# ANRGUSC/DEFER

Hardware: NVIDIA H100
Metric: inferences_per_sec (higher is better)
Workload: dtype bf16x3->f32

## Files before the change

### defer_b200/csrc/conv_umma.cu

```cuda
#include <cuda.h>
#include <string.h>

#include <type_traits>

#include <vector>

#include "common.cuh"
#include "conv_umma.cuh"

namespace defer {

static int env_int(const char* name, int dflt) {
  const char* v = getenv(name);
  return v ? atoi(v) : dflt;
}

namespace {

constexpr int BM = 128;
constexpr int BK = 64;
constexpr int CONS_THREADS = 256;
constexpr int NUM_THREADS = CONS_THREADS + 128;
constexpr int SMEM_CAP = 227 * 1024 - 256;
constexpr int CTL_BYTES = 256;
constexpr int MAX_STAGES = 8;
constexpr int MEGA_BN = 64;
constexpr int STG_COLS = 64;
constexpr int STG_BYTES = BM * STG_COLS * 4;

struct KParams {
  int n, ho, wo, cout;
  int tile_n, tile_h, tile_w, tiles_h, tiles_w;
  int flat;
  int m_total;
  int kh, kw, sh, sw, pad_t, pad_l;
  int cblocks;
  int k_blocks;
  int splits;
  int cluster;
  uint32_t flags;
  const float* scale;
  const float* shift;
  const void* res;
  void* y;
  float* partial;
  unsigned int* counters;
  size_t plane_out;
};

struct alignas(128) MegaOp {
  CUtensorMap tmx[2];
  CUtensorMap tmw[2];
  KParams p;
  int m_tiles, n_tiles;
  const float* stem_x;
  int stem_h, stem_w, stem_cin, stem_kh, stem_kw, stem_sh, stem_sw, stem_pad_t, stem_pad_l, stem_K;
  int stem_win_rows, stem_win_cols;
  const uint8_t* stem_u8;
  float stem_shift[3];
  const float* scale2;
  const float* shift2;
  void* y2;
  int relu2;
  int store_first;
};

template <int NPLANES, int BN>
struct Smem {
  static constexpr int A_PLANE = BM * 128;
  static constexpr int B_PLANE = BN * 128;
  static constexpr int STAGE = NPLANES * (A_PLANE + B_PLANE);
  static constexpr int RED = BM * BN * 4;
  __host__ __device__ static constexpr int ring(int stages, bool red) {
    return (red && stages * STAGE < RED) ? RED : stages * STAGE;
  }
  __host__ __device__ static constexpr int total(int stages, bool red) {
    return ring(stages, red) + STG_BYTES + CTL_BYTES + 1024;
  }
  __host__ __device__ static constexpr int max_stages() {
    return (SMEM_CAP - STG_BYTES - CTL_BYTES - 1024) / STAGE > MAX_STAGES ? MAX_STAGES
                                                                          : (SMEM_CAP - STG_BYTES - CTL_BYTES - 1024) / STAGE;
  }
};
static_assert(Smem<2, 128>::max_stages() == 3 && Smem<2, 64>::max_stages() == 4, "BF16X2 ring depths");
static_assert(Smem<1, 64>::max_stages() == 8 && Smem<1, 128>::max_stages() == 6, "BF16 ring depths");

__device__ __forceinline__ uint32_t smem_u32(const void* p) { return (uint32_t)__cvta_generic_to_shared(p); }

__device__ __forceinline__ void mbar_init(uint32_t bar, uint32_t count) {
  asm volatile("mbarrier.init.shared::cta.b64 [%0], %1;" ::"r"(bar), "r"(count));
}
__device__ __forceinline__ void mbar_arrive_expect_tx(uint32_t bar, uint32_t bytes) {
  asm volatile("mbarrier.arrive.expect_tx.shared::cta.b64 _, [%0], %1;" ::"r"(bar), "r"(bytes) : "memory");
}
__device__ __forceinline__ void mbar_expect_tx(uint32_t bar, uint32_t bytes) {
  asm volatile("mbarrier.expect_tx.relaxed.cta.shared::cta.b64 [%0], %1;" ::"r"(bar), "r"(bytes) : "memory");
}
__device__ __forceinline__ void mbar_arrive(uint32_t bar) {
  asm volatile("mbarrier.arrive.shared::cta.b64 _, [%0];" ::"r"(bar) : "memory");
}
__device__ __forceinline__ bool mbar_try_wait(uint32_t bar, uint32_t parity) {
  uint32_t ok;
  asm volatile(
      "{\n.reg .pred p;\n"
      "mbarrier.try_wait.parity.shared::cta.b64 p, [%1], %2;\n"
      "selp.u32 %0, 1, 0, p;\n}\n"
      : "=r"(ok)
      : "r"(bar), "r"(parity)
      : "memory");
  return ok != 0;
}
__device__ __forceinline__ unsigned long long gtimer() {
  unsigned long long t;
  asm volatile("mov.u64 %0, %%globaltimer;" : "=l"(t));
  return t;
}
__device__ int g_conv_wait_timeout_tag;
__device__ __forceinline__ void mbar_wait(uint32_t bar, uint32_t parity, int tag) {
  if (mbar_try_wait(bar, parity)) return;
  unsigned long long t0 = gtimer();
  unsigned spins = 0;
  while (!mbar_try_wait(bar, parity)) {
    if ((++spins & 0xfff) == 0 && gtimer() - t0 > 2000000000ull) {
      g_conv_wait_timeout_tag = tag;
      asm volatile("trap;");
    }
  }
}

__device__ __forceinline__ void tma_load_4d(uint32_t dst, const CUtensorMap* map, uint32_t bar, int c0, int c1, int c2,
                                            int c3) {
  asm volatile(
      "cp.async.bulk.tensor.4d.shared::cluster.global.mbarrier::complete_tx::bytes [%0], [%1, {%3, %4, %5, %6}], [%2];"
      ::"r"(dst), "l"(reinterpret_cast<uint64_t>(map)), "r"(bar), "r"(c0), "r"(c1), "r"(c2), "r"(c3)
      : "memory");
}
__device__ __forceinline__ void tma_load_3d(uint32_t dst, const CUtensorMap* map, uint32_t bar, int c0, int c1, int c2) {
  asm volatile(
      "cp.async.bulk.tensor.3d.shared::cluster.global.mbarrier::complete_tx::bytes [%0], [%1, {%3, %4, %5}], [%2];"
      ::"r"(dst), "l"(reinterpret_cast<uint64_t>(map)), "r"(bar), "r"(c0), "r"(c1), "r"(c2)
      : "memory");
}

__device__ __forceinline__ void cluster_sync_all() {
  asm volatile("barrier.cluster.arrive.release.aligned;" ::: "memory");
  asm volatile("barrier.cluster.wait.acquire.aligned;" ::: "memory");
}
__device__ __forceinline__ uint32_t cluster_ctarank() {
  uint32_t r;
  asm volatile("mov.u32 %0, %%cluster_ctarank;" : "=r"(r));
  return r;
}
__device__ __forceinline__ uint32_t cluster_nctarank() {
  uint32_t r;
  asm volatile("mov.u32 %0, %%cluster_nctarank;" : "=r"(r));
  return r;
}
__device__ __forceinline__ uint32_t dsmem_map(uint32_t local_addr, uint32_t rank) {
  uint32_t r;
  asm volatile("mapa.shared::cluster.u32 %0, %1, %2;" : "=r"(r) : "r"(local_addr), "r"(rank));
  return r;
}
__device__ __forceinline__ float4 dsmem_ld4(uint32_t addr) {
  float4 v;
  asm volatile("ld.shared::cluster.v4.f32 {%0, %1, %2, %3}, [%4];" : "=f"(v.x), "=f"(v.y), "=f"(v.z), "=f"(v.w) : "r"(addr));
  return v;
}
__device__ __forceinline__ void cons_bar_sync() { asm volatile("bar.sync 1, 256;" ::: "memory"); }
__device__ __forceinline__ void prod_bar_sync() { asm volatile("bar.sync 2, 128;" ::: "memory"); }

__device__ __forceinline__ uint64_t make_sw128_desc(uint32_t smem_addr) {
  return (uint64_t)((smem_addr & 0x3FFFF) >> 4) | (1ull << 16) | (64ull << 32) | (1ull << 62);
}
__device__ __forceinline__ void wg_fence() { asm volatile("wgmma.fence.sync.aligned;" ::: "memory"); }
__device__ __forceinline__ void wg_commit() { asm volatile("wgmma.commit_group.sync.aligned;" ::: "memory"); }
template <int N>
__device__ __forceinline__ void wg_wait() {
  asm volatile("wgmma.wait_group.sync.aligned %0;" ::"n"(N) : "memory");
}
template <int R>
__device__ __forceinline__ void acc_fence(float (&d)[R]) {
#pragma unroll
  for (int i = 0; i < R; ++i) asm volatile("" : "+f"(d[i])::"memory");
}

template <int BN>
__device__ __forceinline__ void wgmma_bf16(float (&d)[BN / 2], uint64_t a, uint64_t b);

template <>
__device__ __forceinline__ void wgmma_bf16<64>(float (&d)[32], uint64_t a, uint64_t b) {
  asm volatile(
      "{\n.reg .pred p;\nsetp.ne.b32 p, %34, 0;\n"
      "wgmma.mma_async.sync.aligned.m64n64k16.f32.bf16.bf16 "
      "{%0, %1, %2, %3, %4, %5, %6, %7, %8, %9, %10, %11, %12, %13, %14, %15, %16, %17, %18, %19, %20, %21, %22, "
      "%23, %24, %25, %26, %27, %28, %29, %30, %31}, %32, %33, p, 1, 1, 0, 0;\n}\n"
      : "+f"(d[0]), "+f"(d[1]), "+f"(d[2]), "+f"(d[3]), "+f"(d[4]), "+f"(d[5]), "+f"(d[6]), "+f"(d[7]), "+f"(d[8]),
        "+f"(d[9]), "+f"(d[10]), "+f"(d[11]), "+f"(d[12]), "+f"(d[13]), "+f"(d[14]), "+f"(d[15]), "+f"(d[16]),
        "+f"(d[17]), "+f"(d[18]), "+f"(d[19]), "+f"(d[20]), "+f"(d[21]), "+f"(d[22]), "+f"(d[23]), "+f"(d[24]),
        "+f"(d[25]), "+f"(d[26]), "+f"(d[27]), "+f"(d[28]), "+f"(d[29]), "+f"(d[30]), "+f"(d[31])
      : "l"(a), "l"(b), "r"(1));
}

template <>
__device__ __forceinline__ void wgmma_bf16<128>(float (&d)[64], uint64_t a, uint64_t b) {
  asm volatile(
      "{\n.reg .pred p;\nsetp.ne.b32 p, %66, 0;\n"
      "wgmma.mma_async.sync.aligned.m64n128k16.f32.bf16.bf16 "
      "{%0, %1, %2, %3, %4, %5, %6, %7, %8, %9, %10, %11, %12, %13, %14, %15, %16, %17, %18, %19, %20, %21, %22, "
      "%23, %24, %25, %26, %27, %28, %29, %30, %31, %32, %33, %34, %35, %36, %37, %38, %39, %40, %41, %42, %43, %44, "
      "%45, %46, %47, %48, %49, %50, %51, %52, %53, %54, %55, %56, %57, %58, %59, %60, %61, %62, %63}, %64, %65, p, "
      "1, 1, 0, 0;\n}\n"
      : "+f"(d[0]), "+f"(d[1]), "+f"(d[2]), "+f"(d[3]), "+f"(d[4]), "+f"(d[5]), "+f"(d[6]), "+f"(d[7]), "+f"(d[8]),
        "+f"(d[9]), "+f"(d[10]), "+f"(d[11]), "+f"(d[12]), "+f"(d[13]), "+f"(d[14]), "+f"(d[15]), "+f"(d[16]),
        "+f"(d[17]), "+f"(d[18]), "+f"(d[19]), "+f"(d[20]), "+f"(d[21]), "+f"(d[22]), "+f"(d[23]), "+f"(d[24]),
        "+f"(d[25]), "+f"(d[26]), "+f"(d[27]), "+f"(d[28]), "+f"(d[29]), "+f"(d[30]), "+f"(d[31]), "+f"(d[32]),
        "+f"(d[33]), "+f"(d[34]), "+f"(d[35]), "+f"(d[36]), "+f"(d[37]), "+f"(d[38]), "+f"(d[39]), "+f"(d[40]),
        "+f"(d[41]), "+f"(d[42]), "+f"(d[43]), "+f"(d[44]), "+f"(d[45]), "+f"(d[46]), "+f"(d[47]), "+f"(d[48]),
        "+f"(d[49]), "+f"(d[50]), "+f"(d[51]), "+f"(d[52]), "+f"(d[53]), "+f"(d[54]), "+f"(d[55]), "+f"(d[56]),
        "+f"(d[57]), "+f"(d[58]), "+f"(d[59]), "+f"(d[60]), "+f"(d[61]), "+f"(d[62]), "+f"(d[63])
      : "l"(a), "l"(b), "r"(1));
}

__device__ __forceinline__ void row_to_pixel(const KParams& p, int r, int n0, int h0, int w0, bool& valid, size_t& pix) {
  if (p.flat) {
    const int m = w0 + r;
    valid = m < p.m_total;
    pix = (size_t)m;
  } else {
    const int tw = r % p.tile_w;
    const int t2 = r / p.tile_w;
    const int th = t2 % p.tile_h;
    const int tn = t2 / p.tile_h;
    const int nn = n0 + tn, oh = h0 + th, ow = w0 + tw;
    valid = (tn < p.tile_n) && nn < p.n && oh < p.ho && ow < p.wo;
    pix = ((size_t)nn * p.ho + oh) * p.wo + ow;
  }
}

struct EpiArgs {
  const float* scale;
  const float* shift;
  const __nv_bfloat16* res;
  __nv_bfloat16* y;
  size_t plane;
  int cout;
  bool relu;
  bool store_first;
  bool relu2;
  const float* scale2;
  const float* shift2;
  __nv_bfloat16* y2;
};

__device__ __forceinline__ EpiArgs epi_args(const MegaOp& op) {
  const KParams& p = op.p;
  EpiArgs e;
  e.scale = p.scale;
  e.shift = p.shift;
  e.res = reinterpret_cast<const __nv_bfloat16*>(p.res);
  e.y = reinterpret_cast<__nv_bfloat16*>(p.y);
  e.plane = p.plane_out;
  e.cout = p.cout;
  e.relu = (p.flags & DEFER_FLAG_RELU) != 0;
  e.store_first = op.store_first != 0;
  e.relu2 = op.relu2 != 0;
  e.scale2 = op.scale2;
  e.shift2 = op.shift2;
  e.y2 = reinterpret_cast<__nv_bfloat16*>(op.y2);
  return e;
}

__device__ __forceinline__ uint32_t stg_off(int r, int c) {
  return (uint32_t)(r * STG_COLS + (((c >> 2) ^ ((r & 7) << 1)) << 2) + (c & 3)) * 4u;
}
__device__ __forceinline__ void sts2(uint32_t addr, float a, float b) {
  asm volatile("st.shared.v2.f32 [%0], {%1, %2};" ::"r"(addr), "f"(a), "f"(b));
}
__device__ __forceinline__ float4 lds4(uint32_t addr) {
  float4 v;
  asm volatile("ld.shared.v4.f32 {%0, %1, %2, %3}, [%4];" : "=f"(v.x), "=f"(v.y), "=f"(v.z), "=f"(v.w) : "r"(addr));
  return v;
}
__device__ __forceinline__ void stg4(void* p, uint4 v) {
  asm volatile("st.global.v4.b32 [%0], {%1, %2, %3, %4};" ::"l"(p), "r"(v.x), "r"(v.y), "r"(v.z), "r"(v.w));
}

__device__ __forceinline__ float bf_lo(uint32_t w) { return __uint_as_float(w << 16); }
__device__ __forceinline__ float bf_hi(uint32_t w) { return __uint_as_float(w & 0xffff0000u); }

template <int NPLANES, int BN, bool AFF>
__device__ __forceinline__ void epi_tile(const KParams& p, const EpiArgs& e, uint32_t stg, const float (&acc)[BN / 2],
                                         uint32_t qmask, int c_base, int n0, int h0, int w0) {
  const int tid = threadIdx.x;
  const int lane = tid & 31;
  const int row0 = (tid >> 7) * 64 + ((tid >> 5) & 3) * 16 + (lane >> 2);
  const int col_l = 2 * (lane & 3);
  const int jg = tid & 7;
  const int rb = tid >> 3;
  const int ca = 2 * jg + ((jg >> 2) & 1), cb = ca ^ 1;
  const bool swap = (jg >> 2) & 1;
  size_t orow[4];
  uint32_t vmask = 0;
#pragma unroll
  for (int k = 0; k < 4; ++k) {
    bool v;
    size_t pix;
    row_to_pixel(p, rb + 32 * k, n0, h0, w0, v, pix);
    orow[k] = pix * (size_t)e.cout;
    vmask |= (uint32_t)v << k;
  }
#pragma unroll
  for (int P = 0; P < BN / STG_COLS; ++P) {
    const bool mine = (qmask >> (8 * P + jg)) & 1u;
    const int c = c_base + STG_COLS * P + 8 * jg;
    cons_bar_sync();
#pragma unroll
    for (int qq = 0; qq < 8; ++qq) {
      const int q = 8 * P + qq;
      if (!((qmask >> q) & 1u)) continue;
      sts2(stg + stg_off(row0, 8 * qq + col_l), acc[4 * q], acc[4 * q + 1]);
      sts2(stg + stg_off(row0 + 8, 8 * qq + col_l), acc[4 * q + 2], acc[4 * q + 3]);
    }
    uint4 rh[4], rl[4];
#pragma unroll
    for (int k = 0; k < 4; ++k) {
      rh[k] = rl[k] = make_uint4(0u, 0u, 0u, 0u);
      if (e.res && mine && ((vmask >> k) & 1u)) {
        rh[k] = __ldcg(reinterpret_cast<const uint4*>(e.res + orow[k] + c));
        if (NPLANES == 2) rl[k] = __ldcg(reinterpret_cast<const uint4*>(e.res + e.plane + orow[k] + c));
      }
    }
    float sc[8], sf[8];
#pragma unroll
    for (int i = 0; i < 8; ++i) { sc[i] = 1.f; sf[i] = 0.f; }
    if (mine) {
      if (e.scale) {
        const float4 a = __ldg(reinterpret_cast<const float4*>(e.scale + c));
        const float4 b = __ldg(reinterpret_cast<const float4*>(e.scale + c + 4));
        sc[0] = a.x; sc[1] = a.y; sc[2] = a.z; sc[3] = a.w; sc[4] = b.x; sc[5] = b.y; sc[6] = b.z; sc[7] = b.w;
      }
      if (e.shift) {
        const float4 a = __ldg(reinterpret_cast<const float4*>(e.shift + c));
        const float4 b = __ldg(reinterpret_cast<const float4*>(e.shift + c + 4));
        sf[0] = a.x; sf[1] = a.y; sf[2] = a.z; sf[3] = a.w; sf[4] = b.x; sf[5] = b.y; sf[6] = b.z; sf[7] = b.w;
      }
    }
    cons_bar_sync();
    if (!mine) continue;

#pragma unroll
    for (int k = 0; k < 4; ++k) {
      if (!((vmask >> k) & 1u)) continue;
      const int r = rb + 32 * k;
      const float4 xa = lds4(stg + stg_off(r, 4 * ca));
      const float4 xb = lds4(stg + stg_off(r, 4 * cb));
      const float4 x0 = swap ? xb : xa, x1 = swap ? xa : xb;
      float v[8] = {x0.x, x0.y, x0.z, x0.w, x1.x, x1.y, x1.z, x1.w};
      const uint32_t hw[4] = {rh[k].x, rh[k].y, rh[k].z, rh[k].w};
      const uint32_t lw[4] = {rl[k].x, rl[k].y, rl[k].z, rl[k].w};
#pragma unroll
      for (int i = 0; i < 8; ++i) {
        v[i] = fmaf(v[i], sc[i], sf[i]);
        if (e.res) {
          v[i] += (i & 1) ? bf_hi(hw[i >> 1]) : bf_lo(hw[i >> 1]);
          if (NPLANES == 2) v[i] += (i & 1) ? bf_hi(lw[i >> 1]) : bf_lo(lw[i >> 1]);
        }
        if (e.relu) v[i] = fmaxf(v[i], 0.f);
      }
      uint4 hi, lo = make_uint4(0u, 0u, 0u, 0u);
      if (NPLANES == 2) {
        split_bf16x2(v[0], v[1], hi.x, lo.x);
        split_bf16x2(v[2], v[3], hi.y, lo.y);
        split_bf16x2(v[4], v[5], hi.z, lo.z);
        split_bf16x2(v[6], v[7], hi.w, lo.w);
      } else {
        hi = make_uint4(pack_bf16x2(v[0], v[1]), pack_bf16x2(v[2], v[3]), pack_bf16x2(v[4], v[5]), pack_bf16x2(v[6], v[7]));
      }
      const size_t o = orow[k] + c;
      if (!AFF || e.store_first) {
        stg4(e.y + o, hi);
        if (NPLANES == 2) stg4(e.y + e.plane + o, lo);
      }
      if constexpr (AFF) {
        float s2[8], t2[8];
        {
          const float4 a = __ldg(reinterpret_cast<const float4*>(e.scale2 + c));
          const float4 b = __ldg(reinterpret_cast<const float4*>(e.scale2 + c + 4));
          const float4 d = __ldg(reinterpret_cast<const float4*>(e.shift2 + c));
          const float4 f = __ldg(reinterpret_cast<const float4*>(e.shift2 + c + 4));
          s2[0] = a.x; s2[1] = a.y; s2[2] = a.z; s2[3] = a.w; s2[4] = b.x; s2[5] = b.y; s2[6] = b.z; s2[7] = b.w;
          t2[0] = d.x; t2[1] = d.y; t2[2] = d.z; t2[3] = d.w; t2[4] = f.x; t2[5] = f.y; t2[6] = f.z; t2[7] = f.w;
        }
        const uint32_t sh[4] = {hi.x, hi.y, hi.z, hi.w};
        const uint32_t sl[4] = {lo.x, lo.y, lo.z, lo.w};
        float u[8];
#pragma unroll
        for (int i = 0; i < 8; ++i) {
          u[i] = (i & 1) ? bf_hi(sh[i >> 1]) : bf_lo(sh[i >> 1]);
          if (NPLANES == 2) u[i] = u[i] + ((i & 1) ? bf_hi(sl[i >> 1]) : bf_lo(sl[i >> 1]));
          u[i] = fmaf(u[i], s2[i], t2[i]);
          if (e.relu2) u[i] = fmaxf(u[i], 0.f);
        }
        uint4 h2, l2;
        if (NPLANES == 2) {
          split_bf16x2(u[0], u[1], h2.x, l2.x);
          split_bf16x2(u[2], u[3], h2.y, l2.y);
          split_bf16x2(u[4], u[5], h2.z, l2.z);
          split_bf16x2(u[6], u[7], h2.w, l2.w);
          stg4(e.y2 + o, h2);
          stg4(e.y2 + e.plane + o, l2);
        } else {
          h2 = make_uint4(pack_bf16x2(u[0], u[1]), pack_bf16x2(u[2], u[3]), pack_bf16x2(u[4], u[5]), pack_bf16x2(u[6], u[7]));
          stg4(e.y2 + o, h2);
        }
      }
    }
  }
}

template <int NPLANES, int BN, int MODE, bool AFF = false>
__device__ __forceinline__ void conv_body(const MegaOp* ops, int n_ops, int stages, int pdl) {
  using L = Smem<NPLANES, BN>;
  constexpr int R = BN / 2;
  extern __shared__ uint8_t smem_raw[];
  uint8_t* smem = reinterpret_cast<uint8_t*>((reinterpret_cast<uintptr_t>(smem_raw) + 1023) & ~(uintptr_t)1023);
  const uint32_t ring = smem_u32(smem);
  const bool red = MODE == 0 && ops[0].p.cluster;
  const uint32_t stg = ring + L::ring(stages, red);
  const uint32_t bar_base = stg + STG_BYTES;
  auto full_bar = [&](int s) { return bar_base + 8u * s; };
  auto empty_bar = [&](int s) { return bar_base + 8u * (stages + s); };
  __shared__ int s_is_last;

  const int tid = threadIdx.x;
  if (tid == 0) {
    for (int s = 0; s < stages; ++s) {
      mbar_init(full_bar(s), 1);
      mbar_init(empty_bar(s), CONS_THREADS / 32);
    }
    asm volatile("fence.mbarrier_init.release.cluster;" ::: "memory");
  }
  __syncthreads();
  if (pdl) {
    asm volatile("griddepcontrol.wait;" ::: "memory");
    asm volatile("griddepcontrol.launch_dependents;" ::: "memory");
  }

  uint32_t it = 0;
  for (int o = 0; o < n_ops; ++o) {
    const MegaOp& op = ops[o];
    const KParams& p = op.p;
    const int total = op.m_tiles * op.n_tiles;
    int t_first, t_step;
    if (MODE == 0) {
      t_first = blockIdx.y * op.m_tiles + blockIdx.x;
      t_step = total;
    } else if (MODE == 1) {
      t_first = blockIdx.x;
      t_step = gridDim.x;
    } else {
      t_first = (int)cluster_ctarank();
      t_step = (int)cluster_nctarank();
    }
    const int split = MODE == 0 ? (int)blockIdx.z : 0;
    const int kb_begin = (split * p.k_blocks) / p.splits;
    const int kb_end = ((split + 1) * p.k_blocks) / p.splits;

    for (int t = t_first; t < total; t += t_step) {
      const int m_tile = t % op.m_tiles;
      const int c_base = (t / op.m_tiles) * BN;
      int n0 = 0, h0 = 0, w0 = 0;
      if (p.flat) {
        w0 = m_tile * BM;
      } else {
        const int tw = m_tile % p.tiles_w;
        const int t2 = m_tile / p.tiles_w;
        n0 = (t2 / p.tiles_h) * p.tile_n;
        h0 = (t2 % p.tiles_h) * p.tile_h;
        w0 = tw * p.tile_w;
      }

      if (tid >= CONS_THREADS) {
        if (tid == CONS_THREADS) {
          const uint32_t a_rows = p.flat ? (uint32_t)BM : (uint32_t)(p.tile_n * p.tile_h * p.tile_w);
          uint32_t i2 = it;
          for (int kb = kb_begin; kb < kb_end; ++kb, ++i2) {
            const int stage = (int)(i2 % (uint32_t)stages);
            const uint32_t phase = (i2 / (uint32_t)stages) & 1u;
            mbar_wait(empty_bar(stage), phase ^ 1u, 1);
            const uint32_t a_dst = ring + stage * L::STAGE;
            const uint32_t b_dst = a_dst + NPLANES * L::A_PLANE;
            const int tap = kb / p.cblocks;
            const int cb = kb - tap * p.cblocks;
            const int khi = tap / p.kw;
            const int kwi = tap - khi * p.kw;
            int cw = w0, ch = 0, cn = 0;
            if (!p.flat) {
              cw = w0 * p.sw + kwi - p.pad_l;
              ch = h0 * p.sh + khi - p.pad_t;
              cn = n0;
            }
            mbar_arrive_expect_tx(full_bar(stage), NPLANES * (a_rows * 128u + (uint32_t)L::B_PLANE));
            tma_load_4d(a_dst, &op.tmx[0], full_bar(stage), cb * BK, cw, ch, cn);
            tma_load_3d(b_dst, &op.tmw[0], full_bar(stage), cb * BK, c_base, tap);
            if (NPLANES == 2) {
              tma_load_4d(a_dst + L::A_PLANE, &op.tmx[1], full_bar(stage), cb * BK, cw, ch, cn);
              tma_load_3d(b_dst + L::B_PLANE, &op.tmw[1], full_bar(stage), cb * BK, c_base, tap);
            }
          }
        }
        it += (uint32_t)(kb_end - kb_begin);
        continue;
      }

      const int wg = tid >> 7;
      const int lane = tid & 31;
      float acc[R];
#pragma unroll
      for (int i = 0; i < R; ++i) acc[i] = 0.f;
      int prev_stage = -1;
      for (int kb = kb_begin; kb < kb_end; ++kb, ++it) {
        const int stage = (int)(it % (uint32_t)stages);
        mbar_wait(full_bar(stage), (it / (uint32_t)stages) & 1u, 2);
        const uint32_t a_addr = ring + stage * L::STAGE + wg * (64 * 128);
        const uint32_t b_addr = ring + stage * L::STAGE + NPLANES * L::A_PLANE;
        wg_fence();
#pragma unroll
        for (int k = 0; k < BK / 16; ++k) {
          const uint64_t a_hi = make_sw128_desc(a_addr + k * 32);
          const uint64_t b_hi = make_sw128_desc(b_addr + k * 32);
          wgmma_bf16<BN>(acc, a_hi, b_hi);
          if (NPLANES == 2) {
            wgmma_bf16<BN>(acc, make_sw128_desc(a_addr + L::A_PLANE + k * 32), b_hi);
            wgmma_bf16<BN>(acc, a_hi, make_sw128_desc(b_addr + L::B_PLANE + k * 32));
          }
        }
        wg_commit();
        wg_wait<1>();
        acc_fence(acc);
        if (prev_stage >= 0 && lane == 0) mbar_arrive(empty_bar(prev_stage));
        prev_stage = stage;
      }
      wg_wait<0>();
      acc_fence(acc);
      if (prev_stage >= 0 && lane == 0) mbar_arrive(empty_bar(prev_stage));


      if (MODE == 0 && p.cluster) {
        cons_bar_sync();
        float4* red_buf = reinterpret_cast<float4*>(smem);
#pragma unroll
        for (int q = 0; q < R / 4; ++q)
          red_buf[q * CONS_THREADS + tid] = make_float4(acc[4 * q], acc[4 * q + 1], acc[4 * q + 2], acc[4 * q + 3]);
        break;
      }
      if (MODE == 0 && p.splits > 1) {
        const size_t tile_lin = (size_t)t;
        float4* mine = reinterpret_cast<float4*>(p.partial) + (tile_lin * p.splits + split) * (R / 4) * CONS_THREADS;
#pragma unroll
        for (int q = 0; q < R / 4; ++q)
          __stcg(mine + q * CONS_THREADS + tid, make_float4(acc[4 * q], acc[4 * q + 1], acc[4 * q + 2], acc[4 * q + 3]));
        __threadfence();
        cons_bar_sync();
        if (tid == 0) {
          const unsigned prev = atomicAdd(p.counters + tile_lin, 1u);
          const int last = prev == (unsigned)(p.splits - 1);
          if (last) p.counters[tile_lin] = 0;
          s_is_last = last;
        }
        cons_bar_sync();
        if (!s_is_last) continue;
        __threadfence();
#pragma unroll
        for (int i = 0; i < R; ++i) acc[i] = 0.f;
        for (int s = 0; s < p.splits; ++s) {
          const float4* src = reinterpret_cast<const float4*>(p.partial) + (tile_lin * p.splits + s) * (R / 4) * CONS_THREADS;
#pragma unroll
          for (int q = 0; q < R / 4; ++q) {
            const float4 v = __ldcg(src + q * CONS_THREADS + tid);
            acc[4 * q] += v.x; acc[4 * q + 1] += v.y; acc[4 * q + 2] += v.z; acc[4 * q + 3] += v.w;
          }
        }
      }
      epi_tile<NPLANES, BN, AFF>(p, epi_args(op), stg, acc, 0xffffu, c_base, n0, h0, w0);
    }

    if (MODE == 0 && p.cluster) {
      cluster_sync_all();
      if (tid < CONS_THREADS) {
        const int m_tile = blockIdx.x;
        int n0 = 0, h0 = 0, w0 = 0;
        if (p.flat) {
          w0 = m_tile * BM;
        } else {
          const int t2 = m_tile / p.tiles_w;
          n0 = (t2 / p.tiles_h) * p.tile_n;
          h0 = (t2 % p.tiles_h) * p.tile_h;
          w0 = (m_tile % p.tiles_w) * p.tile_w;
        }
        const int S = p.splits;
        const int rank = (int)cluster_ctarank();
        const uint32_t mine = ring + (uint32_t)tid * 16u;
        float acc[R];
        uint32_t qmask = 0;
#pragma unroll
        for (int q = 0; q < R / 4; ++q) {
          acc[4 * q] = acc[4 * q + 1] = acc[4 * q + 2] = acc[4 * q + 3] = 0.f;
          if (q % S != rank) continue;
          qmask |= 1u << q;
          const uint32_t addr = mine + (uint32_t)(q * CONS_THREADS) * 16u;
          float4 a = dsmem_ld4(dsmem_map(addr, 0));
          for (int s = 1; s < S; ++s) {
            const float4 v = dsmem_ld4(dsmem_map(addr, (uint32_t)s));
            a.x += v.x; a.y += v.y; a.z += v.z; a.w += v.w;
          }
          acc[4 * q] = a.x; acc[4 * q + 1] = a.y; acc[4 * q + 2] = a.z; acc[4 * q + 3] = a.w;
        }
        epi_tile<NPLANES, BN, AFF>(p, epi_args(op), stg, acc, qmask, (int)blockIdx.y * BN, n0, h0, w0);
      }
      cluster_sync_all();
    }
    if (MODE == 2 && o + 1 < n_ops) {
      asm volatile("fence.proxy.async.global;" ::: "memory");
      cluster_sync_all();
    }
  }
}

template <int NPLANES, int BN>
__global__ void __launch_bounds__(NUM_THREADS, 1) conv_umma_kernel(const __grid_constant__ MegaOp op, int stages, int pdl) {
  conv_body<NPLANES, BN, 0>(&op, 1, stages, pdl);
}

template <int NPLANES, int BN>
__global__ void __launch_bounds__(NUM_THREADS, 1) conv_stream_kernel(const MegaOp* __restrict__ ops, int stages, int pdl) {
  conv_body<NPLANES, BN, 1>(ops, 1, stages, pdl);
}

template <int NPLANES, int BN>
__global__ void __launch_bounds__(NUM_THREADS, 1) conv_umma_aff_kernel(const __grid_constant__ MegaOp op, int stages, int pdl) {
  conv_body<NPLANES, BN, 0, true>(&op, 1, stages, pdl);
}

template <int NPLANES, int BN>
__global__ void __launch_bounds__(NUM_THREADS, 1) conv_stream_aff_kernel(const MegaOp* __restrict__ ops, int stages, int pdl) {
  conv_body<NPLANES, BN, 1, true>(ops, 1, stages, pdl);
}

template <int NPLANES>
__global__ void __launch_bounds__(NUM_THREADS, 1) conv_mega_kernel(const MegaOp* __restrict__ ops, int n_ops, int stages) {
  conv_body<NPLANES, MEGA_BN, 2>(ops, n_ops, stages, 0);
}

enum StemIn { STEM_F32, STEM_U8_CAFFE, STEM_U8_TF };
constexpr int PROD_THREADS = NUM_THREADS - CONS_THREADS;
constexpr int STEM_WIN_BYTES = 24 * 1024;
constexpr int STEM_WIN_VALS = STEM_WIN_BYTES / 4;
constexpr int STEM_FILL = STEM_WIN_VALS / PROD_THREADS;
constexpr int STEM_TILE_W = 16;

template <int NPLANES>
struct StemSmem {
  static constexpr int STAGE = Smem<NPLANES, 64>::STAGE;
  __host__ __device__ static constexpr int total(int stages) {
    return stages * STAGE + STG_BYTES + 2 * STEM_WIN_BYTES + CTL_BYTES + 1024;
  }
  __host__ __device__ static constexpr int max_stages() {
    return (SMEM_CAP - STG_BYTES - 2 * STEM_WIN_BYTES - CTL_BYTES - 1024) / STAGE > MAX_STAGES
               ? MAX_STAGES
               : (SMEM_CAP - STG_BYTES - 2 * STEM_WIN_BYTES - CTL_BYTES - 1024) / STAGE;
  }
};
static_assert(StemSmem<2>::max_stages() == 3 && StemSmem<1>::max_stages() == 6, "stem ring depths with two image windows");
static_assert(STEM_FILL * PROD_THREADS == STEM_WIN_VALS, "the producer threads cover a whole window");

struct StemGeo {
  const float* x;
  const uint8_t* u8;
  float s0, s1, s2;
  int H, rowlen;
  int cin, sh, sw, pad_t, pad_l;
  int wcols, nwin;
  int run, K;
};

__device__ __forceinline__ StemGeo stem_geo(const MegaOp& op) {
  StemGeo g;
  g.x = op.stem_x;
  g.u8 = op.stem_u8;
  g.s0 = op.stem_shift[0]; g.s1 = op.stem_shift[1]; g.s2 = op.stem_shift[2];
  g.H = op.stem_h;
  g.rowlen = op.stem_w * op.stem_cin;
  g.cin = op.stem_cin; g.sh = op.stem_sh; g.sw = op.stem_sw; g.pad_t = op.stem_pad_t; g.pad_l = op.stem_pad_l;
  g.wcols = op.stem_win_cols;
  g.nwin = op.stem_win_rows * op.stem_win_cols;
  g.run = op.stem_kw * op.stem_cin;
  g.K = op.stem_K;
  return g;
}

__device__ __forceinline__ void stem_tile_origin(const KParams& p, int m_tile, int& n0, int& h0, int& w0) {
  const int t2 = m_tile / p.tiles_w;
  n0 = t2 / p.tiles_h;
  h0 = (t2 - n0 * p.tiles_h) * p.tile_h;
  w0 = (m_tile - t2 * p.tiles_w) * p.tile_w;
}

template <int IN>
__device__ __forceinline__ void stem_fill_load(const StemGeo& g, int ptid, int n0, int h0, int w0, uint32_t (&raw)[STEM_FILL]) {
  const int ih0 = h0 * g.sh - g.pad_t, col0 = (w0 * g.sw - g.pad_l) * g.cin;
  const size_t img = (size_t)n0 * g.H * g.rowlen;
  const int dq = PROD_THREADS / g.wcols, dm = PROD_THREADS - dq * g.wcols;
  int wr = ptid / g.wcols, wc = ptid - wr * g.wcols;
  int c = wc % 3;
#pragma unroll
  for (int j = 0; j < STEM_FILL; ++j) {
    const int ih = ih0 + wr, col = col0 + wc;
    const bool in = ptid + PROD_THREADS * j < g.nwin && ih >= 0 && ih < g.H && col >= 0 && col < g.rowlen;
    const size_t off = img + (size_t)(ih * g.rowlen + col);
    if constexpr (IN == STEM_F32) raw[j] = in ? __float_as_uint(__ldg(g.x + off)) : 0u;
    else raw[j] = in ? (uint32_t)__ldg(g.u8 + off + (IN == STEM_U8_CAFFE ? 2 - 2 * c : 0)) : 0x100u;
    wr += dq;
    wc += dm;
    if (wc >= g.wcols) { wc -= g.wcols; ++wr; }
    c = c == 0 ? 2 : c - 1;
  }
}

template <int IN>
__device__ __forceinline__ void stem_fill_store(const StemGeo& g, uint32_t win, int ptid, const uint32_t (&raw)[STEM_FILL]) {
  int c = (ptid % g.wcols) % 3;
#pragma unroll
  for (int j = 0; j < STEM_FILL; ++j) {
    const int e = ptid + PROD_THREADS * j;
    if (e < g.nwin) {
      const float b = __fsub_rn(__uint_as_float(0x4B000000u | raw[j]), 8388608.f);
      float v;
      if constexpr (IN == STEM_F32) v = __uint_as_float(raw[j]);
      else if constexpr (IN == STEM_U8_CAFFE) v = raw[j] > 255u ? 0.f : __fadd_rn(b, c == 0 ? g.s0 : (c == 1 ? g.s1 : g.s2));
      else v = raw[j] > 255u ? 0.f : keras_tf_preprocess(b);
      asm volatile("st.shared.f32 [%0], %1;" ::"r"(win + 4u * (uint32_t)e), "f"(v) : "memory");
    }
    c = c == 0 ? 2 : c - 1;
  }
}

template <int NPLANES>
__device__ __forceinline__ void stem_build(const StemGeo& g, uint32_t win, uint32_t a_dst, int r, int row_base, int kb) {
  int k = kb * BK;
  int a = k / g.run, jj = k - a * g.run;
  uint32_t src = win + 4u * (uint32_t)(row_base + a * g.wcols + jj);
  const uint32_t wrap = 4u * (uint32_t)(g.wcols - g.run);
#pragma unroll 1
  for (int ch = 0; ch < 8; ++ch) {
    float v[8];
#pragma unroll
    for (int e = 0; e < 8; ++e) {
      v[e] = 0.f;
      if (k < g.K) asm volatile("ld.shared.f32 %0, [%1];" : "=f"(v[e]) : "r"(src));
      ++k;
      src += 4u;
      if (++jj == g.run) { jj = 0; src += wrap; }
    }
    const uint32_t off = (uint32_t)r * 128u + ((uint32_t)(ch ^ (r & 7)) << 4);
    uint32_t h[4], l[4];
#pragma unroll
    for (int q = 0; q < 4; ++q) {
      if (NPLANES == 2) split_bf16x2(v[2 * q], v[2 * q + 1], h[q], l[q]);
      else h[q] = pack_bf16x2(v[2 * q], v[2 * q + 1]);
    }
    asm volatile("st.shared.v4.b32 [%0], {%1, %2, %3, %4};" ::"r"(a_dst + off), "r"(h[0]), "r"(h[1]), "r"(h[2]), "r"(h[3])
                 : "memory");
    if (NPLANES == 2)
      asm volatile("st.shared.v4.b32 [%0], {%1, %2, %3, %4};" ::"r"(a_dst + Smem<NPLANES, 64>::A_PLANE + off), "r"(l[0]),
                   "r"(l[1]), "r"(l[2]), "r"(l[3])
                   : "memory");
  }
}

template <int NPLANES, int IN>
__device__ __forceinline__ void stem_body(const MegaOp* ops, int stages, int pdl) {
  using L = Smem<NPLANES, 64>;
  extern __shared__ uint8_t smem_raw[];
  uint8_t* smem = reinterpret_cast<uint8_t*>((reinterpret_cast<uintptr_t>(smem_raw) + 1023) & ~(uintptr_t)1023);
  const uint32_t ring = smem_u32(smem);
  const uint32_t stg = ring + stages * L::STAGE;
  const uint32_t win0 = stg + STG_BYTES;
  const uint32_t bar_base = win0 + 2 * STEM_WIN_BYTES;
  auto full_bar = [&](int s) { return bar_base + 8u * s; };
  auto empty_bar = [&](int s) { return bar_base + 8u * (stages + s); };

  const int tid = threadIdx.x;
  if (tid == 0) {
    for (int s = 0; s < stages; ++s) {
      mbar_init(full_bar(s), 1);
      mbar_init(empty_bar(s), CONS_THREADS / 32);
    }
    asm volatile("fence.mbarrier_init.release.cluster;" ::: "memory");
  }
  __syncthreads();
  if (pdl) {
    asm volatile("griddepcontrol.wait;" ::: "memory");
    asm volatile("griddepcontrol.launch_dependents;" ::: "memory");
  }

  const MegaOp& op = ops[0];
  const KParams& p = op.p;
  const int total = op.m_tiles * op.n_tiles;
  const int k_blocks = p.k_blocks;
  uint32_t it = 0;

  if (tid >= CONS_THREADS) {
    const int ptid = tid - CONS_THREADS;
    const StemGeo g = stem_geo(op);
    int th = ptid / p.tile_w, tw = ptid - th * p.tile_w;
    if (th >= p.tile_h) th = tw = 0;
    const int row_base = th * g.sh * g.wcols + tw * g.sw * g.cin;
    uint32_t raw[STEM_FILL];
    int n0, h0, w0;
    if ((int)blockIdx.x < total) {
      stem_tile_origin(p, (int)blockIdx.x % op.m_tiles, n0, h0, w0);
      stem_fill_load<IN>(g, ptid, n0, h0, w0, raw);
      stem_fill_store<IN>(g, win0, ptid, raw);
    }
    int wb = 0;
    for (int t = blockIdx.x; t < total; t += gridDim.x, wb ^= 1) {
      const int t_next = t + (int)gridDim.x;
      if (t_next < total) {
        stem_tile_origin(p, t_next % op.m_tiles, n0, h0, w0);
        stem_fill_load<IN>(g, ptid, n0, h0, w0, raw);
      }
      prod_bar_sync();
      const uint32_t win = win0 + (uint32_t)wb * STEM_WIN_BYTES;
      const int c_base = (t / op.m_tiles) * 64;
      for (int kb = 0; kb < k_blocks; ++kb, ++it) {
        const int stage = (int)(it % (uint32_t)stages);
        mbar_wait(empty_bar(stage), ((it / (uint32_t)stages) & 1u) ^ 1u, 1);
        const uint32_t a_dst = ring + stage * L::STAGE;
        const uint32_t b_dst = a_dst + NPLANES * L::A_PLANE;
        if (ptid == 0) {
          mbar_expect_tx(full_bar(stage), NPLANES * (uint32_t)L::B_PLANE);
          tma_load_3d(b_dst, &op.tmw[0], full_bar(stage), kb * BK, c_base, 0);
          if (NPLANES == 2) tma_load_3d(b_dst + L::B_PLANE, &op.tmw[1], full_bar(stage), kb * BK, c_base, 0);
        }
        stem_build<NPLANES>(g, win, a_dst, ptid, row_base, kb);
        asm volatile("fence.proxy.async.shared::cta;" ::: "memory");
        prod_bar_sync();
        if (ptid == 0) mbar_arrive(full_bar(stage));
      }
      if (t_next < total) stem_fill_store<IN>(g, win0 + (uint32_t)(wb ^ 1) * STEM_WIN_BYTES, ptid, raw);
    }
    return;
  }

  const int wg = tid >> 7;
  const int lane = tid & 31;
  for (int t = blockIdx.x; t < total; t += gridDim.x) {
    float acc[32];
#pragma unroll
    for (int i = 0; i < 32; ++i) acc[i] = 0.f;
    int prev_stage = -1;
    for (int kb = 0; kb < k_blocks; ++kb, ++it) {
      const int stage = (int)(it % (uint32_t)stages);
      mbar_wait(full_bar(stage), (it / (uint32_t)stages) & 1u, 2);
      const uint32_t a_addr = ring + stage * L::STAGE + wg * (64 * 128);
      const uint32_t b_addr = ring + stage * L::STAGE + NPLANES * L::A_PLANE;
      wg_fence();
#pragma unroll
      for (int k = 0; k < BK / 16; ++k) {
        const uint64_t a_hi = make_sw128_desc(a_addr + k * 32);
        const uint64_t b_hi = make_sw128_desc(b_addr + k * 32);
        wgmma_bf16<64>(acc, a_hi, b_hi);
        if (NPLANES == 2) {
          wgmma_bf16<64>(acc, make_sw128_desc(a_addr + L::A_PLANE + k * 32), b_hi);
          wgmma_bf16<64>(acc, a_hi, make_sw128_desc(b_addr + L::B_PLANE + k * 32));
        }
      }
      wg_commit();
      wg_wait<1>();
      acc_fence(acc);
      if (prev_stage >= 0 && lane == 0) mbar_arrive(empty_bar(prev_stage));
      prev_stage = stage;
    }
    wg_wait<0>();
    acc_fence(acc);
    if (prev_stage >= 0 && lane == 0) mbar_arrive(empty_bar(prev_stage));
    int n0, h0, w0;
    stem_tile_origin(p, t % op.m_tiles, n0, h0, w0);
    epi_tile<NPLANES, 64, false>(p, epi_args(op), stg, acc, 0xffffu, (t / op.m_tiles) * 64, n0, h0, w0);
  }
}

template <int NPLANES>
__global__ void __launch_bounds__(NUM_THREADS, 1) conv_stem_kernel(const MegaOp* __restrict__ ops, int stages, int pdl) {
  stem_body<NPLANES, STEM_F32>(ops, stages, pdl);
}

template <int NPLANES>
__global__ void __launch_bounds__(NUM_THREADS, 1) conv_stem_u8_kernel(const MegaOp* __restrict__ ops, int stages, int pdl) {
  stem_body<NPLANES, STEM_U8_CAFFE>(ops, stages, pdl);
}

template <int NPLANES>
__global__ void __launch_bounds__(NUM_THREADS, 1) conv_stem_u8tf_kernel(const MegaOp* __restrict__ ops, int stages, int pdl) {
  stem_body<NPLANES, STEM_U8_TF>(ops, stages, pdl);
}

__global__ void __launch_bounds__(256) weight_transform_kernel(const float* __restrict__ w, __nv_bfloat16* __restrict__ out,
                                                               int taps, int cin, int cout, int nplanes) {
  size_t total = (size_t)taps * cin * cout;
  size_t i = (size_t)blockIdx.x * blockDim.x + threadIdx.x;
  if (i >= total) return;
  int ci = (int)(i % cin);
  size_t t2 = i / cin;
  int co = (int)(t2 % cout);
  int tap = (int)(t2 / cout);
  float v = w[((size_t)tap * cin + ci) * cout + co];
  __nv_bfloat16 hi = __float2bfloat16_rn(v);
  out[i] = hi;
  if (nplanes == 2) out[total + i] = __float2bfloat16_rn(v - __bfloat162float(hi));
}

typedef CUresult (*PFN_encodeTiled)(CUtensorMap*, CUtensorMapDataType, cuuint32_t, void*, const cuuint64_t*,
                                    const cuuint64_t*, const cuuint32_t*, const cuuint32_t*, CUtensorMapInterleave,
                                    CUtensorMapSwizzle, CUtensorMapL2promotion, CUtensorMapFloatOOBfill);

PFN_encodeTiled get_encode() {
  static PFN_encodeTiled fn = nullptr;
  if (!fn) {
    void* p = nullptr;
    cudaDriverEntryPointQueryResult q;
    if (cudaGetDriverEntryPoint("cuTensorMapEncodeTiled", &p, cudaEnableDefault, &q) == cudaSuccess &&
        q == cudaDriverEntryPointSuccess)
      fn = (PFN_encodeTiled)p;
  }
  return fn;
}

int encode_map(CUtensorMap* map, void* base, int rank, const uint64_t* dims, const uint64_t* strides_bytes,
               const uint32_t* box, const uint32_t* estr) {
  PFN_encodeTiled enc = get_encode();
  if (!enc) {
    set_error("cuTensorMapEncodeTiled entry point not available");
    return DEFER_ERR_CUDA;
  }
  CUresult r = enc(map, CU_TENSOR_MAP_DATA_TYPE_BFLOAT16, (cuuint32_t)rank, base, (const cuuint64_t*)dims,
                   (const cuuint64_t*)strides_bytes, (const cuuint32_t*)box, (const cuuint32_t*)estr,
                   CU_TENSOR_MAP_INTERLEAVE_NONE, CU_TENSOR_MAP_SWIZZLE_128B, CU_TENSOR_MAP_L2_PROMOTION_L2_256B,
                   CU_TENSOR_MAP_FLOAT_OOB_FILL_NONE);
// ... 471 lines not shown
```

Measured before the change: 14240.

## Add dedicated persistent stream body with decoupled producer and prefetched residuals

Replaces the persistent-grid path with a specialized stream_body. In it the TMA producer thread runs ahead across all tiles without per-tile synchronisation, and registers are rebalanced between producer and consumer warpgroups via setmaxnreg. Consumers load the residual tile into registers before the MMA main loop, so the global-load latency overlaps the MMA work instead of sitting in the epilogue. This costs extra register pressure from holding the residual tile, and the epilogue assumes every column quad is owned by a thread (qmask is all ones).

```diff
diff --git a/defer_b200/csrc/conv_umma.cu b/defer_b200/csrc/conv_umma.cu
--- a/defer_b200/csrc/conv_umma.cu
+++ b/defer_b200/csrc/conv_umma.cu
@@ -288,9 +288,41 @@
 __device__ __forceinline__ float bf_lo(uint32_t w) { return __uint_as_float(w << 16); }
 __device__ __forceinline__ float bf_hi(uint32_t w) { return __uint_as_float(w & 0xffff0000u); }
 
+__device__ __forceinline__ uint32_t epi_rows(const KParams& p, int cout, int tid, int n0, int h0, int w0, size_t (&orow)[4]) {
+  uint32_t vmask = 0;
+#pragma unroll
+  for (int k = 0; k < 4; ++k) {
+    bool v;
+    size_t pix;
+    row_to_pixel(p, (tid >> 3) + 32 * k, n0, h0, w0, v, pix);
+    orow[k] = pix * (size_t)cout;
+    vmask |= (uint32_t)v << k;
+  }
+  return vmask;
+}
+
+template <int NPLANES>
+__device__ __forceinline__ void epi_res_load(const EpiArgs& e, const size_t (&orow)[4], uint32_t vmask, int c, bool mine,
+                                             uint4 (&rh)[4], uint4 (&rl)[4]) {
+#pragma unroll
+  for (int k = 0; k < 4; ++k) {
+    rh[k] = rl[k] = make_uint4(0u, 0u, 0u, 0u);
+    if (e.res && mine && ((vmask >> k) & 1u)) {
+      rh[k] = __ldcg(reinterpret_cast<const uint4*>(e.res + orow[k] + c));
+      if (NPLANES == 2) rl[k] = __ldcg(reinterpret_cast<const uint4*>(e.res + e.plane + orow[k] + c));
+    }
+  }
+}
+
+template <int BN>
+struct ResTile {
+  uint4 h[BN / STG_COLS][4], l[BN / STG_COLS][4];
+};
+
 template <int NPLANES, int BN, bool AFF>
 __device__ __forceinline__ void epi_tile(const KParams& p, const EpiArgs& e, uint32_t stg, const float (&acc)[BN / 2],
-                                         uint32_t qmask, int c_base, int n0, int h0, int w0) {
+                                         uint32_t qmask, int c_base, int n0, int h0, int w0,
+                                         const ResTile<BN>* pre = nullptr) {
   const int tid = threadIdx.x;
   const int lane = tid & 31;
   const int row0 = (tid >> 7) * 64 + ((tid >> 5) & 3) * 16 + (lane >> 2);
@@ -300,15 +332,7 @@
   const int ca = 2 * jg + ((jg >> 2) & 1), cb = ca ^ 1;
   const bool swap = (jg >> 2) & 1;
   size_t orow[4];
-  uint32_t vmask = 0;
-#pragma unroll
-  for (int k = 0; k < 4; ++k) {
-    bool v;
-    size_t pix;
-    row_to_pixel(p, rb + 32 * k, n0, h0, w0, v, pix);
-    orow[k] = pix * (size_t)e.cout;
-    vmask |= (uint32_t)v << k;
-  }
+  const uint32_t vmask = epi_rows(p, e.cout, tid, n0, h0, w0, orow);
 #pragma unroll
   for (int P = 0; P < BN / STG_COLS; ++P) {
     const bool mine = (qmask >> (8 * P + jg)) & 1u;
@@ -322,13 +346,14 @@
       sts2(stg + stg_off(row0 + 8, 8 * qq + col_l), acc[4 * q + 2], acc[4 * q + 3]);
     }
     uint4 rh[4], rl[4];
-#pragma unroll
-    for (int k = 0; k < 4; ++k) {
-      rh[k] = rl[k] = make_uint4(0u, 0u, 0u, 0u);
-      if (e.res && mine && ((vmask >> k) & 1u)) {
-        rh[k] = __ldcg(reinterpret_cast<const uint4*>(e.res + orow[k] + c));
-        if (NPLANES == 2) rl[k] = __ldcg(reinterpret_cast<const uint4*>(e.res + e.plane + orow[k] + c));
+    if (pre) {
+#pragma unroll
+      for (int k = 0; k < 4; ++k) {
+        rh[k] = pre->h[P][k];
+        rl[k] = pre->l[P][k];
       }
+    } else {
+      epi_res_load<NPLANES>(e, orow, vmask, c, mine, rh, rl);
     }
     float sc[8], sf[8];
 #pragma unroll
@@ -418,8 +443,93 @@
   }
 }
 
+__device__ __forceinline__ void tile_origin(const MegaOp& op, int t, int bn, int& c_base, int& n0, int& h0, int& w0) {
+  const KParams& p = op.p;
+  const int m_tile = t % op.m_tiles;
+  c_base = (t / op.m_tiles) * bn;
+  n0 = h0 = w0 = 0;
+  if (p.flat) {
+    w0 = m_tile * BM;
+  } else {
+    const int tw = m_tile % p.tiles_w;
+    const int t2 = m_tile / p.tiles_w;
+    n0 = (t2 / p.tiles_h) * p.tile_n;
+    h0 = (t2 % p.tiles_h) * p.tile_h;
+    w0 = tw * p.tile_w;
+  }
+}
+
+template <int NPLANES, int BN>
+__device__ __forceinline__ void produce_tile(const MegaOp& op, uint32_t ring, uint32_t bar_base, int stages, uint32_t it,
+                                             int kb_begin, int kb_end, int c_base, int n0, int h0, int w0) {
+  using L = Smem<NPLANES, BN>;
+  const KParams& p = op.p;
+  const uint32_t a_rows = p.flat ? (uint32_t)BM : (uint32_t)(p.tile_n * p.tile_h * p.tile_w);
+  for (int kb = kb_begin; kb < kb_end; ++kb, ++it) {
+    const int stage = (int)(it % (uint32_t)stages);
+    const uint32_t phase = (it / (uint32_t)stages) & 1u;
+    const uint32_t full = bar_base + 8u * stage, empty = bar_base + 8u * (stages + stage);
+    mbar_wait(empty, phase ^ 1u, 1);
+    const uint32_t a_dst = ring + stage * L::STAGE;
+    const uint32_t b_dst = a_dst + NPLANES * L::A_PLANE;
+    const int tap = kb / p.cblocks;
+    const int cb = kb - tap * p.cblocks;
+    const int khi = tap / p.kw;
+    const int kwi = tap - khi * p.kw;
+    int cw = w0, ch = 0, cn = 0;
+    if (!p.flat) {
+      cw = w0 * p.sw + kwi - p.pad_l;
+      ch = h0 * p.sh + khi - p.pad_t;
+      cn = n0;
+    }
+    mbar_arrive_expect_tx(full, NPLANES * (a_rows * 128u + (uint32_t)L::B_PLANE));
+    tma_load_4d(a_dst, &op.tmx[0], full, cb * BK, cw, ch, cn);
+    tma_load_3d(b_dst, &op.tmw[0], full, cb * BK, c_base, tap);
+    if (NPLANES == 2) {
+      tma_load_4d(a_dst + L::A_PLANE, &op.tmx[1], full, cb * BK, cw, ch, cn);
+      tma_load_3d(b_dst + L::B_PLANE, &op.tmw[1], full, cb * BK, c_base, tap);
+    }
+  }
+}
+
+template <int NPLANES, int BN>
+__device__ __forceinline__ void consume_tile(uint32_t ring, uint32_t bar_base, int stages, uint32_t& it, int n_kb, int wg,
+                                             float (&acc)[BN / 2], int wait_tag) {
+  using L = Smem<NPLANES, BN>;
+  const int lane = threadIdx.x & 31;
+#pragma unroll
+  for (int i = 0; i < BN / 2; ++i) acc[i] = 0.f;
+  int prev_stage = -1;
+  for (int kb = 0; kb < n_kb; ++kb, ++it) {
+    const int stage = (int)(it % (uint32_t)stages);
+    mbar_wait(bar_base + 8u * stage, (it / (uint32_t)stages) & 1u, wait_tag);
+    const uint32_t a_addr = ring + stage * L::STAGE + wg * (64 * 128);
+    const uint32_t b_addr = ring + stage * L::STAGE + NPLANES * L::A_PLANE;
+    wg_fence();
+#pragma unroll
+    for (int k = 0; k < BK / 16; ++k) {
+      const uint64_t a_hi = make_sw128_desc(a_addr + k * 32);
+      const uint64_t b_hi = make_sw128_desc(b_addr + k * 32);
+      wgmma_bf16<BN>(acc, a_hi, b_hi);
+      if (NPLANES == 2) {
+        wgmma_bf16<BN>(acc, make_sw128_desc(a_addr + L::A_PLANE + k * 32), b_hi);
+        wgmma_bf16<BN>(acc, a_hi, make_sw128_desc(b_addr + L::B_PLANE + k * 32));
+      }
+    }
+    wg_commit();
+    wg_wait<1>();
+    acc_fence(acc);
+    if (prev_stage >= 0 && lane == 0) mbar_arrive(bar_base + 8u * (stages + prev_stage));
+    prev_stage = stage;
+  }
+  wg_wait<0>();
+  acc_fence(acc);
+  if (prev_stage >= 0 && lane == 0) mbar_arrive(bar_base + 8u * (stages + prev_stage));
+}
+
 template <int NPLANES, int BN, int MODE, bool AFF = false>
 __device__ __forceinline__ void conv_body(const MegaOp* ops, int n_ops, int stages, int pdl) {
+  static_assert(MODE == 0 || MODE == 2, "the persistent grid is stream_body");
   using L = Smem<NPLANES, BN>;
   constexpr int R = BN / 2;
   extern __shared__ uint8_t smem_raw[];
@@ -455,9 +565,6 @@
     if (MODE == 0) {
       t_first = blockIdx.y * op.m_tiles + blockIdx.x;
       t_step = total;
-    } else if (MODE == 1) {
-      t_first = blockIdx.x;
-      t_step = gridDim.x;
     } else {
       t_first = (int)cluster_ctarank();
       t_step = (int)cluster_nctarank();
@@ -467,83 +574,18 @@
     const int kb_end = ((split + 1) * p.k_blocks) / p.splits;
 
     for (int t = t_first; t < total; t += t_step) {
-      const int m_tile = t % op.m_tiles;
-      const int c_base = (t / op.m_tiles) * BN;
-      int n0 = 0, h0 = 0, w0 = 0;
-      if (p.flat) {
-        w0 = m_tile * BM;
-      } else {
-        const int tw = m_tile % p.tiles_w;
-        const int t2 = m_tile / p.tiles_w;
-        n0 = (t2 / p.tiles_h) * p.tile_n;
-        h0 = (t2 % p.tiles_h) * p.tile_h;
-        w0 = tw * p.tile_w;
-      }
+      int c_base, n0, h0, w0;
+      tile_origin(op, t, BN, c_base, n0, h0, w0);
 
       if (tid >= CONS_THREADS) {
-        if (tid == CONS_THREADS) {
-          const uint32_t a_rows = p.flat ? (uint32_t)BM : (uint32_t)(p.tile_n * p.tile_h * p.tile_w);
-          uint32_t i2 = it;
-          for (int kb = kb_begin; kb < kb_end; ++kb, ++i2) {
-            const int stage = (int)(i2 % (uint32_t)stages);
-            const uint32_t phase = (i2 / (uint32_t)stages) & 1u;
-            mbar_wait(empty_bar(stage), phase ^ 1u, 1);
-            const uint32_t a_dst = ring + stage * L::STAGE;
-            const uint32_t b_dst = a_dst + NPLANES * L::A_PLANE;
-            const int tap = kb / p.cblocks;
-            const int cb = kb - tap * p.cblocks;
-            const int khi = tap / p.kw;
-            const int kwi = tap - khi * p.kw;
-            int cw = w0, ch = 0, cn = 0;
-            if (!p.flat) {
-              cw = w0 * p.sw + kwi - p.pad_l;
-              ch = h0 * p.sh + khi - p.pad_t;
-              cn = n0;
-            }
-            mbar_arrive_expect_tx(full_bar(stage), NPLANES * (a_rows * 128u + (uint32_t)L::B_PLANE));
-            tma_load_4d(a_dst, &op.tmx[0], full_bar(stage), cb * BK, cw, ch, cn);
-            tma_load_3d(b_dst, &op.tmw[0], full_bar(stage), cb * BK, c_base, tap);
-            if (NPLANES == 2) {
-              tma_load_4d(a_dst + L::A_PLANE, &op.tmx[1], full_bar(stage), cb * BK, cw, ch, cn);
-              tma_load_3d(b_dst + L::B_PLANE, &op.tmw[1], full_bar(stage), cb * BK, c_base, tap);
-            }
-          }
-        }
+        if (tid == CONS_THREADS)
+          produce_tile<NPLANES, BN>(op, ring, bar_base, stages, it, kb_begin, kb_end, c_base, n0, h0, w0);
         it += (uint32_t)(kb_end - kb_begin);
         continue;
       }
 
-      const int wg = tid >> 7;
-      const int lane = tid & 31;
       float acc[R];
-#pragma unroll
-      for (int i = 0; i < R; ++i) acc[i] = 0.f;
-      int prev_stage = -1;
-      for (int kb = kb_begin; kb < kb_end; ++kb, ++it) {
-        const int stage = (int)(it % (uint32_t)stages);
-        mbar_wait(full_bar(stage), (it / (uint32_t)stages) & 1u, 2);
-        const uint32_t a_addr = ring + stage * L::STAGE + wg * (64 * 128);
-        const uint32_t b_addr = ring + stage * L::STAGE + NPLANES * L::A_PLANE;
-        wg_fence();
-#pragma unroll
-        for (int k = 0; k < BK / 16; ++k) {
-          const uint64_t a_hi = make_sw128_desc(a_addr + k * 32);
-          const uint64_t b_hi = make_sw128_desc(b_addr + k * 32);
-          wgmma_bf16<BN>(acc, a_hi, b_hi);
-          if (NPLANES == 2) {
-            wgmma_bf16<BN>(acc, make_sw128_desc(a_addr + L::A_PLANE + k * 32), b_hi);
-            wgmma_bf16<BN>(acc, a_hi, make_sw128_desc(b_addr + L::B_PLANE + k * 32));
-          }
-        }
-        wg_commit();
-        wg_wait<1>();
-        acc_fence(acc);
-        if (prev_stage >= 0 && lane == 0) mbar_arrive(empty_bar(prev_stage));
-        prev_stage = stage;
-      }
-      wg_wait<0>();
-      acc_fence(acc);
-      if (prev_stage >= 0 && lane == 0) mbar_arrive(empty_bar(prev_stage));
+      consume_tile<NPLANES, BN>(ring, bar_base, stages, it, kb_end - kb_begin, tid >> 7, acc, 2);
 
 
       if (MODE == 0 && p.cluster) {
@@ -627,6 +669,66 @@
   }
 }
 
+template <int NPLANES, int BN, bool AFF>
+__device__ __forceinline__ void stream_body(const MegaOp* ops, int stages, int pdl) {
+  using L = Smem<NPLANES, BN>;
+  extern __shared__ uint8_t smem_raw[];
+  uint8_t* smem = reinterpret_cast<uint8_t*>((reinterpret_cast<uintptr_t>(smem_raw) + 1023) & ~(uintptr_t)1023);
+  const uint32_t ring = smem_u32(smem);
+  const uint32_t stg = ring + L::ring(stages, false);
+  const uint32_t bar_base = stg + STG_BYTES;
+
+  const int tid = threadIdx.x;
+  if (tid == 0) {
+    for (int s = 0; s < stages; ++s) {
+      mbar_init(bar_base + 8u * s, 1);
+      mbar_init(bar_base + 8u * (stages + s), CONS_THREADS / 32);
+    }
+    asm volatile("fence.mbarrier_init.release.cluster;" ::: "memory");
+  }
+  __syncthreads();
+  if (pdl) {
+    asm volatile("griddepcontrol.wait;" ::: "memory");
+    asm volatile("griddepcontrol.launch_dependents;" ::: "memory");
+  }
+
+  const MegaOp& op = ops[0];
+  const KParams& p = op.p;
+  const int total = op.m_tiles * op.n_tiles;
+  const int n_kb = p.k_blocks;
+  uint32_t it = 0;
+
+  if (tid >= CONS_THREADS) {
+    asm volatile("setmaxnreg.dec.sync.aligned.u32 40;" ::: "memory");
+    if (tid == CONS_THREADS) {
+      for (int t = blockIdx.x; t < total; t += gridDim.x, it += (uint32_t)n_kb) {
+        int c_base, n0, h0, w0;
+        tile_origin(op, t, BN, c_base, n0, h0, w0);
+        produce_tile<NPLANES, BN>(op, ring, bar_base, stages, it, 0, n_kb, c_base, n0, h0, w0);
+      }
+    }
+    return;
+  }
+
+  asm volatile("setmaxnreg.inc.sync.aligned.u32 232;" ::: "memory");
+  for (int t = blockIdx.x; t < total; t += gridDim.x) {
+    int c_base, n0, h0, w0;
+    tile_origin(op, t, BN, c_base, n0, h0, w0);
+    const EpiArgs e = epi_args(op);
+    ResTile<BN> res;
+    {
+      size_t orow[4];
+      const uint32_t vmask = epi_rows(p, e.cout, tid, n0, h0, w0, orow);
+#pragma unroll
+      for (int P = 0; P < BN / STG_COLS; ++P)
+        epi_res_load<NPLANES>(e, orow, vmask, c_base + STG_COLS * P + 8 * (tid & 7), true, res.h[P], res.l[P]);
+    }
+    float acc[BN / 2];
+    consume_tile<NPLANES, BN>(ring, bar_base, stages, it, n_kb, tid >> 7, acc, 3);
+    epi_tile<NPLANES, BN, AFF>(p, e, stg, acc, 0xffffu, c_base, n0, h0, w0, &res);
+  }
+}
+
 template <int NPLANES, int BN>
 __global__ void __launch_bounds__(NUM_THREADS, 1) conv_umma_kernel(const __grid_constant__ MegaOp op, int stages, int pdl) {
   conv_body<NPLANES, BN, 0>(&op, 1, stages, pdl);
@@ -634,7 +736,7 @@
 
 template <int NPLANES, int BN>
 __global__ void __launch_bounds__(NUM_THREADS, 1) conv_stream_kernel(const MegaOp* __restrict__ ops, int stages, int pdl) {
-  conv_body<NPLANES, BN, 1>(ops, 1, stages, pdl);
+  stream_body<NPLANES, BN, false>(ops, stages, pdl);
 }
 
 template <int NPLANES, int BN>
@@ -644,7 +746,7 @@
 
 template <int NPLANES, int BN>
 __global__ void __launch_bounds__(NUM_THREADS, 1) conv_stream_aff_kernel(const MegaOp* __restrict__ ops, int stages, int pdl) {
-  conv_body<NPLANES, BN, 1, true>(ops, 1, stages, pdl);
+  stream_body<NPLANES, BN, true>(ops, stages, pdl);
 }
 
 template <int NPLANES>
```

After: 14710, median of 6. +3.3%, better.
